# Project-Arda/bgls

Measured on AMD Instinct MI355X. Metric: aggregate-verify signer-pairs/sec, higher is better.
Workload: dtype u32; 1 GPU; altbn128 VerifyAggregateSignature, one 1048576-signer batch, keys+msgs resident in HBM; curve=altbn128, signers=1048576, signers_per_gpu=1048576, in_flight=8

## Files before the change

### bgls_amd/csrc/constants_gen.hpp

```cpp
#pragma once
#include <stdint.h>

namespace bgls {

struct BN254 {
  static constexpr int L = 8;
  static constexpr int CURVE_ID = 0;
  static constexpr bool TWIST_D = true;
  static constexpr int FP_BYTES = 32;
  static constexpr uint32_t N0INV = 0xe4866389u;
  static constexpr int XI_RE = 9;
  static constexpr uint32_t P[8] = {0xd87cfd47u, 0x3c208c16u, 0x6871ca8du, 0x97816a91u, 0x8181585du, 0xb85045b6u, 0xe131a029u, 0x30644e72u};
  static constexpr uint32_t P2W[16] = {0x275d69b1u, 0x3b5458a2u, 0x09eac101u, 0xa602072du, 0x6d96cadcu, 0x4a50189cu, 0x7a1242c8u, 0x04689e95u, 0x34c6b38du, 0x26edfa5cu, 0x16375606u, 0xb00b8551u, 0x0348d21cu, 0x599a6f7cu, 0x763cbf9cu, 0x0925c4b8u};
  static constexpr uint32_t P2W3[16] = {0x76183d13u, 0xb1fd09e6u, 0x1dc04303u, 0xf2061587u, 0x48c46095u, 0xdef049d5u, 0x6e36c858u, 0x0d39dbc0u, 0x9e541aa7u, 0x74c9ef14u, 0x42a60212u, 0x10228ff3u, 0x09da7656u, 0x0ccf4e74u, 0x62b63ed5u, 0x1b714e29u};
  static constexpr uint32_t P2W6[16] = {0xec307a26u, 0x63fa13ccu, 0x3b808607u, 0xe40c2b0eu, 0x9188c12bu, 0xbde093aau, 0xdc6d90b1u, 0x1a73b780u, 0x3ca8354eu, 0xe993de29u, 0x854c0424u, 0x20451fe6u, 0x13b4ecacu, 0x199e9ce8u, 0xc56c7daau, 0x36e29c52u};
  static constexpr uint32_t ONE[8] = {0xc58f0d9du, 0xd35d438du, 0xf5c70b3du, 0x0a78eb28u, 0x7879462cu, 0x666ea36fu, 0x9a07df2fu, 0x0e0a77c1u};
  static constexpr uint32_t R2[8] = {0x538afa89u, 0xf32cfc5bu, 0xd44501fbu, 0xb5e71911u, 0x0a417ff6u, 0x47ab1effu, 0xcab8351fu, 0x06d89f71u};
  static constexpr uint32_t HALF[8] = {0x4f060572u, 0x87bee7d2u, 0x2f1c6ae5u, 0xd0fd2addu, 0xfcfd4f44u, 0x8f5f7492u, 0x3d9cbfacu, 0x1f37631au};
  static constexpr uint32_t B[8] = {0x50ad28d7u, 0x7a17caa9u, 0xe15521b9u, 0x1f6ac17au, 0x696bd284u, 0x334bea4eu, 0xce179d8eu, 0x2a1f6744u};
  static constexpr uint32_t B2_RE[8] = {0x77b802a8u, 0x3bf938e3u, 0x3633535du, 0x020b1b27u, 0x49755260u, 0x26b7edf0u, 0x4384a86du, 0x2514c632u};
  static constexpr uint32_t B2_IM[8] = {0xd1dcff67u, 0x38e7ecccu, 0x93ce0d3eu, 0x65f0b37du, 0x22ac00aau, 0xd749d0ddu, 0x4a688d4du, 0x0141b9ceu};
  static constexpr uint32_t B2X3_RE[8] = {0xb62e0d6au, 0x3baa927cu, 0xd1b664fdu, 0xd71e7c52u, 0xd95d4664u, 0x03873e63u, 0x082ab8f4u, 0x0e75b5b1u};
  static constexpr uint32_t B2X3_IM[8] = {0x7596fe35u, 0xaab7c666u, 0xbb6a27bau, 0x31d21a78u, 0x680401ffu, 0x85dd7297u, 0xdf39a7e9u, 0x03c52d6au};
  static constexpr uint32_t GAMMA[288] = {0xc58f0d9du, 0xd35d438du, 0xf5c70b3du, 0x0a78eb28u, 0x7879462cu, 0x666ea36fu, 0x9a07df2fu, 0x0e0a77c1u, 0x00000000u, 0x00000000u, 0x00000000u, 0x00000000u, 0x00000000u, 0x00000000u, 0x00000000u, 0x00000000u, 0x33144907u, 0xaf9ba696u, 0x87afb78au, 0xca6b1d73u, 0xf08a2087u, 0x11bded5eu, 0x1a1f3a7cu, 0x02f34d75u, 0x4c492d72u, 0xa222ae23u, 0x565de15bu, 0xd00f02a4u, 0x53dfc926u, 0xdc2ff3a2u, 0xb3899551u, 0x10a75716u, 0x4563ab30u, 0xb5773b10u, 0xa9aa6454u, 0x347f91c8u, 0x242e0991u, 0x7a007127u, 0x118214ecu, 0x1956bcd8u, 0xa0aa4757u, 0x6e849f1eu, 0x89f89141u, 0xaa1c7b6du, 0xfae0ca3au, 0xb6e713cdu, 0x4e82ebc3u, 0x26694fbbu, 0x2936b629u, 0xe4bbdd0cu, 0xe133bacbu, 0xbb30f162u, 0xf9645366u, 0x31a9d1b6u, 0xa500f8ddu, 0x253570beu, 0x5ffe77c7u, 0xa1d77ce4u, 0x7826d1dbu, 0x07affd11u, 0xbb7edc6bu, 0x6d16bd27u, 0x85defeccu, 0x2c872002u, 0x843abe92u, 0x7361d77fu, 0x273411fbu, 0xa5bb2bd3u, 0x4b3e2399u, 0x9c941f31u, 0xbb9fd3ecu, 0x15df9cddu, 0x4bd8c949u, 0x5dddfd15u, 0xa4445b60u, 0x62cb29a5u, 0x0c7dd2b9u, 0x37bc870au, 0x3171f0fdu, 0x24830a9du, 0x41690fe7u, 0xc970692fu, 0x27694b0bu, 0xe2403421u, 0x83c459e8u, 0x32bee66bu, 0x0ab08841u, 0x12aabcedu, 0x40aebfa9u, 0x0d485d23u, 0xab2fcc57u, 0x05193418u, 0x8a4910f5u, 0xd3b0a40bu, 0x35d2925au, 0x2f21ebb5u, 0xc58f0d9du, 0xd35d438du, 0xf5c70b3du, 0x0a78eb28u, 0x7879462cu, 0x666ea36fu, 0x9a07df2fu, 0x0e0a77c1u, 0x00000000u, 0x00000000u, 0x00000000u, 0x00000000u, 0x00000000u, 0x00000000u, 0x00000000u, 0x00000000u, 0x00fa1bf2u, 0xca8d8005u, 0x68b39769u, 0xf0c5d614u, 0xad0d4418u, 0x0e201271u, 0xbad856e6u, 0x04290f65u, 0x00000000u, 0x00000000u, 0x00000000u, 0x00000000u, 0x00000000u, 0x00000000u, 0x00000000u, 0x00000000u, 0x13e80b9cu, 0x3350c88eu, 0xdb5e56b9u, 0x7dce557cu, 0xb615564au, 0x6001b4b8u, 0x020217e0u, 0x2682e617u, 0x00000000u, 0x00000000u, 0x00000000u, 0x00000000u, 0x00000000u, 0x00000000u, 0x00000000u, 0x00000000u, 0x12edefaau, 0x68c34889u, 0x72aabf4fu, 0x8d087f68u, 0x09081231u, 0x51e1a247u, 0x4729c0fau, 0x2259d6b1u, 0x00000000u, 0x00000000u, 0x00000000u, 0x00000000u, 0x00000000u, 0x00000000u, 0x00000000u, 0x00000000u, 0xd782e155u, 0x71930c11u, 0xffbe3323u, 0xa6bb947cu, 0xd4741444u, 0xaa303344u, 0x26594943u, 0x2c3b3f0du, 0x00000000u, 0x00000000u, 0x00000000u, 0x00000000u, 0x00000000u, 0x00000000u, 0x00000000u, 0x00000000u, 0xc494f1abu, 0x08cfc388u, 0x8d1373d4u, 0x19b31514u, 0xcb6c0213u, 0x584e90fdu, 0xdf2f8849u, 0x09e1685bu, 0x00000000u, 0x00000000u, 0x00000000u, 0x00000000u, 0x00000000u, 0x00000000u, 0x00000000u, 0x00000000u, 0xc58f0d9du, 0xd35d438du, 0xf5c70b3du, 0x0a78eb28u, 0x7879462cu, 0x666ea36fu, 0x9a07df2fu, 0x0e0a77c1u, 0x00000000u, 0x00000000u, 0x00000000u, 0x00000000u, 0x00000000u, 0x00000000u, 0x00000000u, 0x00000000u, 0x4e46d97du, 0x36531618u, 0xd4c96d9fu, 0x0af7129eu, 0xca1009b5u, 0x659da72fu, 0x83a20d23u, 0x08116d89u, 0xc39c1939u, 0xb1df4af7u, 0x8a73bf7fu, 0x3d9f0287u, 0x8caf0ae0u, 0x9b222092u, 0xeff054a6u, 0x26684515u, 0x16ad6badu, 0xc9af22f7u, 0x4aa662b2u, 0xb311782au, 0xe248c7f4u, 0x19eeaf64u, 0xe3439f82u, 0x20273e77u, 0xf7ce93acu, 0xacc02860u, 0x7ba76b4cu, 0x3933d581u, 0x446c8467u, 0x69e6188bu, 0x4417cc55u, 0x0a46036du, 0xaf46471eu, 0x5764af0au, 0x873e0fc1u, 0xdc50792eu, 0x881d04f6u, 0x86a673ffu, 0x3c30a74cu, 0x0b2eddb4u, 0x787e8580u, 0x9a490f32u, 0xf04af8b1u, 0x8fd16d7fu, 0xc6027bf2u, 0x4b39888eu, 0x5b52a15du, 0x03dd2e70u, 0x7b6762dfu, 0x448a93a5u, 0x28fdeadfu, 0xbfd62df5u, 0x0e9bd47au, 0xd858f5d0u, 0x3476ec58u, 0x06b03d4du, 0xbcc936d1u, 0x2b19daf4u, 0x56f4299fu, 0xa1a54e7au, 0x5adeaef1u, 0xb533eee0u, 0x84dda0b2u, 0x170c812bu, 0x75cf559fu, 0xe0bc4b22u, 0xc154e60fu, 0xc238b945u, 0x929a7d5eu, 0x803982a5u, 0xf7e4a37eu, 0x15ce052du, 0xbf3799a7u, 0x2d28efbdu, 0x1ad60773u, 0x9b097e3cu, 0xaf4a535bu, 0x982d4113u, 0xe3056063u, 0x24e18991u};
// ... 109 lines not shown
  static constexpr uint32_t RX_B2_RE[14] = {0x0d1ff2e0u, 0x06000000u, 0x000ac467u, 0x03379b48u, 0x01c84b80u, 0x00e88243u, 0x00dd9a7eu, 0x0683dcf8u, 0x06c26d0bu, 0x04a5eec2u, 0x0457663cu, 0x004b29f1u, 0x0967f3e8u, 0x00015de9u};
  static constexpr uint32_t RX_B2_IM[14] = {0x0d1ff2e0u, 0x06000000u, 0x000ac467u, 0x03379b48u, 0x01c84b80u, 0x00e88243u, 0x00dd9a7eu, 0x0683dcf8u, 0x06c26d0bu, 0x04a5eec2u, 0x0457663cu, 0x004b29f1u, 0x0967f3e8u, 0x00015de9u};
  static constexpr uint32_t RX_GAMMA[112] = {0x00000000u, 0x00000000u, 0x00000000u, 0x00000000u, 0x00000000u, 0x00000000u, 0x00000000u, 0x00000000u, 0x00000000u, 0x00000000u, 0x00000000u, 0x00000000u, 0x00000000u, 0x00000000u, 0x02421b59u, 0x0bee4867u, 0x01d31002u, 0x04760184u, 0x04cc5086u, 0x0c76dc00u, 0x0aae891bu, 0x0ac70ad2u, 0x0fe377c4u, 0x0e4686b8u, 0x05ed1568u, 0x08f5a180u, 0x002b5c1fu, 0x0000d1a4u, 0x033e2f27u, 0x032a25aau, 0x027ca1d2u, 0x0c1e049eu, 0x0c3f707au, 0x0055ca94u, 0x02010b7bu, 0x03b93794u, 0x0d5a86aau, 0x0a544de3u, 0x0556a044u, 0x09c66da5u, 0x038ec515u, 0x0000cea3u, 0x033e2f27u, 0x032a25aau, 0x027ca1d2u, 0x0c1e049eu, 0x0c3f707au, 0x0055ca94u, 0x02010b7bu, 0x03b93794u, 0x0d5a86aau, 0x0a544de3u, 0x0556a044u, 0x09c66da5u, 0x038ec515u, 0x0000cea3u, 0x0a75929au, 0x0681b798u, 0x022a3e9du, 0x0abc02bfu, 0x04e5bb45u, 0x055e6e7eu, 0x04814117u, 0x06d04f1bu, 0x0ae3387du, 0x054acb0cu, 0x00a4c74bu, 0x056138b5u, 0x0b64e066u, 0x000076f2u, 0x00000000u, 0x00000000u, 0x00000000u, 0x00000000u, 0x00000000u, 0x00000000u, 0x00000000u, 0x00000000u, 0x00000000u, 0x00000000u, 0x00000000u, 0x00000000u, 0x00000000u, 0x00000000u, 0x0cb7adf3u, 0x026fffffu, 0x03fd4ea0u, 0x0f320443u, 0x09b20bcbu, 0x01d54a7eu, 0x0f2fca33u, 0x019759edu, 0x0ac6b042u, 0x039151c5u, 0x0691dcb4u, 0x0e56da35u, 0x0b903c85u, 0x00014896u, 0x00000000u, 0x00000000u, 0x00000000u, 0x00000000u, 0x00000000u, 0x00000000u, 0x00000000u, 0x00000000u, 0x00000000u, 0x00000000u, 0x00000000u, 0x00000000u, 0x00000000u, 0x00000000u};
  static constexpr uint32_t RX_PK[126] = {0x00000000u, 0x00000000u, 0x00000000u, 0x00000000u, 0x00000000u, 0x00000000u, 0x00000000u, 0x00000000u, 0x00000000u, 0x00000000u, 0x00000000u, 0x00000000u, 0x00000000u, 0x00000000u, 0x0fffaaabu, 0x0fefffffu, 0x03ffffb9u, 0x0fffeb15u, 0x06241eabu, 0x0a0f6b0fu, 0x0f6730d2u, 0x0f38512bu, 0x04774b84u, 0x04bacd76u, 0x0ba7b643u, 0x0e69a4b1u, 0x01ea397fu, 0x0001a011u, 0x0fff5556u, 0x0fdfffffu, 0x07ffff73u, 0x0fffd62au, 0x0c483d57u, 0x041ed61eu, 0x0ece61a5u, 0x0e70a257u, 0x08ee9709u, 0x09759aecu, 0x074f6c86u, 0x0cd34963u, 0x03d472ffu, 0x00034022u, 0x0fff0001u, 0x0fcfffffu, 0x0bffff2du, 0x0fffc13fu, 0x026c5c03u, 0x0e2e412eu, 0x0e359277u, 0x0da8f383u, 0x0d65e28eu, 0x0e306862u, 0x02f722c9u, 0x0b3cee15u, 0x05beac7fu, 0x0004e033u, 0x0ffeaaacu, 0x0fbfffffu, 0x0ffffee7u, 0x0fffac54u, 0x08907aafu, 0x083dac3du, 0x0d9cc34au, 0x0ce144afu, 0x01dd2e13u, 0x02eb35d9u, 0x0e9ed90du, 0x09a692c6u, 0x07a8e5ffu, 0x00068044u, 0x0ffe5557u, 0x0fafffffu, 0x03fffea1u, 0x0fff976au, 0x0eb4995bu, 0x024d174cu, 0x0d03f41du, 0x0c1995dbu, 0x06547998u, 0x07a6034fu, 0x0a468f50u, 0x08103778u, 0x09931f7fu, 0x00082055u, 0x0ffe0002u, 0x0f9fffffu, 0x07fffe5bu, 0x0fff827fu, 0x04d8b807u, 0x0c5c825cu, 0x0c6b24efu, 0x0b51e707u, 0x0acbc51du, 0x0c60d0c5u, 0x05ee4593u, 0x0679dc2au, 0x0b7d58ffu, 0x0009c066u, 0x0ffdaaadu, 0x0f8fffffu, 0x0bfffe15u, 0x0fff6d94u, 0x0afcd6b3u, 0x066bed6bu, 0x0bd255c2u, 0x0a8a3833u, 0x0f4310a2u, 0x011b9e3bu, 0x0195fbd7u, 0x04e380dcu, 0x0d67927fu, 0x000b6077u, 0x0ffd5558u, 0x0f7fffffu, 0x0ffffdcfu, 0x0fff58a9u, 0x0120f55fu, 0x007b587bu, 0x0b398695u, 0x09c2895fu, 0x03ba5c27u, 0x05d66bb2u, 0x0d3db21au, 0x034d258du, 0x0f51cbffu, 0x000d0088u};
  static constexpr uint32_t RX_LAD[84] = {0x0fff5556u, 0x0fdfffffu, 0x07ffff73u, 0x0fffd62au, 0x0c483d57u, 0x041ed61eu, 0x0ece61a5u, 0x0e70a257u, 0x08ee9709u, 0x09759aecu, 0x074f6c86u, 0x0cd34963u, 0x03d472ffu, 0x00034022u, 0x0ffeaaacu, 0x0fbfffffu, 0x0ffffee7u, 0x0fffac54u, 0x08907aafu, 0x083dac3du, 0x0d9cc34au, 0x0ce144afu, 0x01dd2e13u, 0x02eb35d9u, 0x0e9ed90du, 0x09a692c6u, 0x07a8e5ffu, 0x00068044u, 0x0ffd5558u, 0x0f7fffffu, 0x0ffffdcfu, 0x0fff58a9u, 0x0120f55fu, 0x007b587bu, 0x0b398695u, 0x09c2895fu, 0x03ba5c27u, 0x05d66bb2u, 0x0d3db21au, 0x034d258du, 0x0f51cbffu, 0x000d0088u, 0x0ffaaab0u, 0x0effffffu, 0x0ffffb9fu, 0x0ffeb153u, 0x0241eabfu, 0x00f6b0f6u, 0x06730d2au, 0x038512bfu, 0x0774b84fu, 0x0bacd764u, 0x0a7b6434u, 0x069a4b1bu, 0x0ea397feu, 0x001a0111u, 0x0ff55560u, 0x0dffffffu, 0x0ffff73fu, 0x0ffd62a7u, 0x0483d57fu, 0x01ed61ecu, 0x0ce61a54u, 0x070a257eu, 0x0ee9709eu, 0x0759aec8u, 0x04f6c869u, 0x0d349637u, 0x0d472ffcu, 0x00340223u, 0x0feaaac0u, 0x0bffffffu, 0x0fffee7fu, 0x0ffac54fu, 0x0907aaffu, 0x03dac3d8u, 0x09cc34a8u, 0x0e144afdu, 0x0dd2e13cu, 0x0eb35d91u, 0x09ed90d2u, 0x0a692c6eu, 0x0a8e5ff9u, 0x00680447u};
};

struct BN254W : BN254 {
  static constexpr int RX_NL = 9;
  static constexpr int RX_W = 29;
  static constexpr uint32_t RX_MASK = 0x1fffffffu;
  static constexpr int RX_VBND = 4;
  static constexpr uint32_t RX_P[9] = {0x187cfd47u, 0x010460b6u, 0x1c72a34fu, 0x02d522d0u, 0x1585d978u, 0x02db40c0u, 0x00a6e141u, 0x0e5c2634u, 0x0030644eu};
  static constexpr uint32_t RX_NP = 0x4866389u;
  static constexpr uint32_t RX_ONE[9] = {0x157ccc21u, 0x141c2758u, 0x185230d3u, 0x014c0419u, 0x0aa36fb9u, 0x1d4240ceu, 0x11d54c07u, 0x052ac7a8u, 0x000dc836u};
  static constexpr uint32_t RX_R2[9] = {0x059bac10u, 0x0d1503a3u, 0x018016b8u, 0x10ab0ca8u, 0x02632639u, 0x02c0169fu, 0x169bfd53u, 0x11869d4cu, 0x002a11a6u};
  static constexpr uint32_t RX_TO[9] = {0x13349ca1u, 0x1a5d84a8u, 0x0a3e5cacu, 0x100249e0u, 0x12b951e8u, 0x0e92d304u, 0x14cb95b3u, 0x041b9d3du, 0x00058003u};
  static constexpr uint32_t RX_BACK[8] = {0x00000000u, 0x00000000u, 0x00000000u, 0x00000000u, 0x00000000u, 0x00000000u, 0x00000000u, 0x08000000u};
  static constexpr uint32_t RX_TOM[9] = {0x058f0d9du, 0x1aea1c6eu, 0x11c2cf74u, 0x11d651ebu, 0x1462c0a7u, 0x11b7bc3cu, 0x1cbd99bau, 0x183340fbu, 0x000e0a77u};
  static constexpr int RX_FAT_VB = 1;
  static constexpr int RX_FAT_KMAX = 6;
  static constexpr uint32_t RX_FAT[54] = {0x30f9fa8eu, 0x2208c16cu, 0x38e5469du, 0x25aa45a0u, 0x2b0bb2efu, 0x25b68180u, 0x214dc281u, 0x3cb84c67u, 0x0060c89bu, 0x4976f7d5u, 0x430d2222u, 0x5557e9ebu, 0x487f6870u, 0x40918c66u, 0x4891c240u, 0x41f4a3c1u, 0x4b14729au, 0x00912ce9u, 0x61f3f51cu, 0x641182d8u, 0x71ca8d39u, 0x6b548b40u, 0x761765ddu, 0x6b6d02ffu, 0x629b8501u, 0x797098cdu, 0x00c19136u, 0x9a70f263u, 0x8515e38du, 0x8e3d3087u, 0x8e29ae10u, 0x8b9d3f54u, 0x8e4843bfu, 0x83426641u, 0x87ccbf00u, 0x00f1f584u, 0xb2edefaau, 0xa61a4443u, 0xaaafd3d5u, 0xb0fed0e0u, 0xa12318cbu, 0xb123847fu, 0xa3e94781u, 0xb628e533u, 0x012259d1u, 0xcb6aecf1u, 0xc71ea4f9u, 0xc7227723u, 0xd3d3f3b0u, 0xd6a8f242u, 0xd3fec53eu, 0xc49028c1u, 0xc4850b66u, 0x0152be1fu};
  static constexpr uint64_t RX_BIAS_D3[18] = {0xbffffff6af4933bull, 0x17fffffeaa626d14ull, 0x23fffffdeceed0c9ull, 0x2ffffffd3de78d78ull, 0x3bfffffc65892178ull, 0x47fffffbaf384418ull, 0x53fffffaeef3e68aull, 0x5ffffffa2d17640aull, 0x54912ce7002863abull, 0x48912ce7c0000000ull, 0x3c912ce880000000ull, 0x30912ce940000000ull, 0x24912cea00000000ull, 0x18912ceac0000000ull, 0xc912ceb80000000ull, 0x912cec40000000ull, 0x1b71500000000ull, 0x0ull};
  static constexpr uint64_t RX_BIAS_S6[18] = {0x0ull, 0x0ull, 0x0ull, 0x0ull, 0x0ull, 0x0ull, 0x0ull, 0x0ull, 0x0ull, 0x0ull, 0x0ull, 0x0ull, 0x0ull, 0x0ull, 0x0ull, 0x0ull, 0x0ull, 0x0ull};
  static constexpr uint32_t RX_B2X3_RE[9] = {0x095cc5c1u, 0x016b1649u, 0x13202c16u, 0x05967b15u, 0x0b150904u, 0x0c884f0eu, 0x1423d855u, 0x02e3530fu, 0x001b2ff4u};
  static constexpr uint32_t RX_B2X3_IM[9] = {0x01e5cc12u, 0x15bda508u, 0x18588eb7u, 0x00f3e938u, 0x18f2b0b4u, 0x03bffebeu, 0x13752c37u, 0x0ec49a37u, 0x0017dd10u};
  static constexpr uint32_t RX_B2_RE[9] = {0x0b489658u, 0x00cfd255u, 0x0fdb9a77u, 0x02ce89f7u, 0x0033a0d4u, 0x1a768545u, 0x06ee3ddcu, 0x106a7dc1u, 0x0019316bu};
  static constexpr uint32_t RX_B2_IM[9] = {0x1b9fece0u, 0x07ecccd1u, 0x1069f1c7u, 0x0cdf64f3u, 0x0154cbe1u, 0x0dd22ac0u, 0x06eba4e8u, 0x1929a235u, 0x00283739u};
  static constexpr uint32_t RX_GAMMA[72] = {0x04a59190u, 0x06f504d9u, 0x0bf870bbu, 0x171ffd5cu, 0x1ac4d17du, 0x04be36d5u, 0x0bceec27u, 0x1a83a513u, 0x002492b3u, 0x11142ef1u, 0x0b31acc7u, 0x1d5818bcu, 0x180afc17u, 0x1a63177eu, 0x15765b3bu, 0x118f742eu, 0x063a509au, 0x00135e4eu, 0x1b1f0678u, 0x0373fb06u, 0x13170fbdu, 0x185d74b7u, 0x0241131fu, 0x16e18435u, 0x1ef3b6ceu, 0x01f06f02u, 0x001d46bdu, 0x19a647d5u, 0x19fdefabu, 0x1d925d1au, 0x0d1f6c5fu, 0x08ac6cc5u, 0x1fa5621au, 0x134f06feu, 0x09a72816u, 0x0015871du, 0x18ccb791u, 0x175b1c3au, 0x0b83d6e2u, 0x0e8ed071u, 0x1282bee2u, 0x04220e84u, 0x1fe4017fu, 0x15084d4au, 0x00169119u, 0x00000000u, 0x00000000u, 0x00000000u, 0x00000000u, 0x00000000u, 0x00000000u, 0x00000000u, 0x00000000u, 0x00000000u, 0x03003126u, 0x0ce8395eu, 0x0420727bu, 0x01891eb7u, 0x0ae269bfu, 0x0598fff2u, 0x0ed19539u, 0x09315e8bu, 0x00229c18u, 0x00000000u, 0x00000000u, 0x00000000u, 0x00000000u, 0x00000000u, 0x00000000u, 0x00000000u, 0x00000000u, 0x00000000u};
  static constexpr uint32_t RX_PK[81] = {0x00000000u, 0x00000000u, 0x00000000u, 0x00000000u, 0x00000000u, 0x00000000u, 0x00000000u, 0x00000000u, 0x00000000u, 0x187cfd47u, 0x010460b6u, 0x1c72a34fu, 0x02d522d0u, 0x1585d978u, 0x02db40c0u, 0x00a6e141u, 0x0e5c2634u, 0x0030644eu, 0x10f9fa8eu, 0x0208c16du, 0x18e5469eu, 0x05aa45a1u, 0x0b0bb2f0u, 0x05b68181u, 0x014dc282u, 0x1cb84c68u, 0x0060c89cu, 0x0976f7d5u, 0x030d2224u, 0x1557e9edu, 0x087f6872u, 0x00918c68u, 0x0891c242u, 0x01f4a3c3u, 0x0b14729cu, 0x00912cebu, 0x01f3f51cu, 0x041182dbu, 0x11ca8d3cu, 0x0b548b43u, 0x161765e0u, 0x0b6d0302u, 0x029b8504u, 0x197098d0u, 0x00c19139u, 0x1a70f263u, 0x0515e391u, 0x0e3d308bu, 0x0e29ae14u, 0x0b9d3f58u, 0x0e4843c3u, 0x03426645u, 0x07ccbf04u, 0x00f1f588u, 0x12edefaau, 0x061a4448u, 0x0aafd3dau, 0x10fed0e5u, 0x012318d0u, 0x11238484u, 0x03e94786u, 0x1628e538u, 0x012259d6u, 0x0b6aecf1u, 0x071ea4ffu, 0x07227729u, 0x13d3f3b6u, 0x16a8f248u, 0x13fec544u, 0x049028c7u, 0x04850b6cu, 0x0152be25u, 0x03e7ea38u, 0x082305b6u, 0x03951a78u, 0x16a91687u, 0x0c2ecbc0u, 0x16da0605u, 0x05370a08u, 0x12e131a0u, 0x01832273u};
  static constexpr uint32_t RX_LAD[54] = {0x10f9fa8eu, 0x0208c16du, 0x18e5469eu, 0x05aa45a1u, 0x0b0bb2f0u, 0x05b68181u, 0x014dc282u, 0x1cb84c68u, 0x0060c89cu, 0x01f3f51cu, 0x041182dbu, 0x11ca8d3cu, 0x0b548b43u, 0x161765e0u, 0x0b6d0302u, 0x029b8504u, 0x197098d0u, 0x00c19139u, 0x03e7ea38u, 0x082305b6u, 0x03951a78u, 0x16a91687u, 0x0c2ecbc0u, 0x16da0605u, 0x05370a08u, 0x12e131a0u, 0x01832273u, 0x07cfd470u, 0x10460b6cu, 0x072a34f0u, 0x0d522d0eu, 0x185d9781u, 0x0db40c0au, 0x0a6e1411u, 0x05c26340u, 0x030644e7u, 0x0f9fa8e0u, 0x008c16d8u, 0x0e5469e1u, 0x1aa45a1cu, 0x10bb2f02u, 0x1b681815u, 0x14dc2822u, 0x0b84c680u, 0x060c89ceu, 0x1f3f51c0u, 0x01182db0u, 0x1ca8d3c2u, 0x1548b438u, 0x01765e05u, 0x16d0302bu, 0x09b85045u, 0x17098d01u, 0x0c19139cu};
  static constexpr int64_t RX_XIG0[9] = {844385340ll, 595946497ll, 594944858ll, 816853286ll, 626800348ll, 805628652ll, 767515872ll, 770429518ll, -88799382ll};
  static constexpr int64_t RX_XIG1[9] = {274749216ll, 527690023ll, 296457758ll, 89892323ll, 256168189ll, 77064170ll, 186898397ll, 343619967ll, -101485007ll};
};

}
```

### bgls_amd/csrc/miller_x.hpp

```cpp
#pragma once
#include <type_traits>
#include "dev_common.hpp"
#include "coop.hpp"
#include "rx_pair.hpp"

namespace bgls {

template <class C>
struct MxForm { typedef C type; };
template <>
struct MxForm<BN254> { typedef BN254W type; };

template <class C, int NP = 60, bool XL_ = (std::is_same<C, BN254W>::value && NP == 60)>
struct MX {
  static_assert(NP == 60 || NP == 64, "pairings per block");
  static constexpr bool XL = XL_;
  static_assert(!XL || (NP == 60 && !rx_lazy<C> && C::TWIST_D && C::RX_NL <= 12), "XL: the 29-bit form's 60-pairing block, D-type twist");
  static constexpr int NL = C::RX_NL;
  static constexpr bool PACKED = (C::RX_NL % 4) != 0 && C::CURVE_ID == 1;
  static constexpr int HS = PACKED ? NL : ((NL + 3) & ~3);
  static constexpr int ES = 2 * HS;
  static constexpr int NLINES = NP == 64 ? 7 : 6;
  static constexpr int FOLD_UNROLL = (!rx_lazy<C> && NLINES % 3 == 0) ? 3 : 1;
  static constexpr int KS = PACKED ? 2 * ES : ES;
  static constexpr int WS = XL ? 112 : (PACKED ? 368 : 176);
  static constexpr int GROUP_DW = XL ? 1020 : (PACKED ? (NP == 64 ? 940 : 844) : (NP == 64 ? 828 : 764));
  static constexpr int THREADS = 192;
  static __device__ __forceinline__ int acc_off(int k, int wrap) { return k * KS + wrap * WS; }
  static __device__ __forceinline__ int line_off(int e) {
    if constexpr (PACKED) return e < 12 ? 28 + 56 * e + (e >= 6 ? 32 : 0) : (e == 12 ? 336 : 704 + 28 * (e - 13));
    else return 320 + ES * e;
  }
  static_assert(!PACKED || (ES == 28 && 704 + 28 * (3 * NLINES - 13) <= GROUP_DW), "BLS12-381 line slots");
  static_assert(PACKED || XL || 320 + ES * 3 * NLINES <= GROUP_DW, "alt-bn128 line slots");
  static __device__ __forceinline__ int line_off_x(int m, int t, bool xi, bool glo) {
    return t == 0 ? 256 + ES * m : (t == 1 ? (xi ? 544 + (glo ? 8 : 0) : 400) + ES * m : (xi ? 696 : 840) + ES * m);
  }
  static_assert(!XL || (ES == 24 && KS == 24 && WS + 3 * KS >= 6 * KS && WS + 6 * KS <= 256 && 840 + 6 * ES <= GROUP_DW), "XL line slots");
  static constexpr int PQ = 10 * GROUP_DW;
  static constexpr int P_LDS_LIMIT = 40960;
  static constexpr bool P_IN_LDS = (10 * GROUP_DW + NP * 2 * HS) * 4 <= P_LDS_LIMIT;
  static constexpr int BLOCK_BYTES = (10 * GROUP_DW + (P_IN_LDS ? NP * 2 * HS : 0)) * 4;
  static_assert(!XL || (BLOCK_BYTES <= 40960 && !P_IN_LDS), "XL: four blocks per CU; the hash points' coordinates are parked in the workspace");
  static constexpr int NPARK_Q = C::CURVE_ID == 0 ? 6 : 2;
  static constexpr int NPARK = NPARK_Q + (P_IN_LDS ? 0 : 2);
  static constexpr int PS = (NL + 3) & ~3;
  static constexpr size_t park_bytes(size_t nblocks) { return nblocks * 128 * NPARK * PS * 4; }
};

// ... 306 lines not shown
        const Sx<C, SX_T> b2 = sx_const<C>(odd ? C::RX_B2_IM : C::RX_B2_RE);
        const auto d = sx_sub<C>(pair_sqr<C>(yq, odd), sx_add<C>(pair_mul<C>(pair_sqr<C>(xq, odd), xq, odd), b2));
        const bool on_own = sx_is_zero_mod_p<C>(d);
        const bool on_curve = on_own && pair_swap1(on_own ? 1 : 0) != 0;
        if (valid && !(canon && (qinf || on_curve))) atomicOr(flags, FLAG_ENC);
      }
      Aff<F1<C>> P = g1s[valid ? idx : 0];
      valid = valid && !P.inf && !qinf;
      if (!valid) {
        xq = ux_to_sx<C>(to_ux<C>(fp_load<C>(C::G2 + (odd ? C::L : 0))));
        yq = ux_to_sx<C>(to_ux<C>(fp_load<C>(C::G2 + 2 * C::L + (odd ? C::L : 0))));
        P.x = fp_load<C>(C::G1X);
        P.y = fp_load<C>(C::G1Y);
      }
      MxPark<C>::st(mypark, 0, xq);
      MxPark<C>::st(mypark, 1, yq);
      if constexpr (C::CURVE_ID == 0) {
        const Sx<C, SX_T> cx = sx_select<C>(odd, sx_neg<C>(xq), xq), cy = sx_select<C>(odd, sx_neg<C>(yq), yq);
        constexpr int N2 = 2 * C::RX_NL;
        MxPark<C>::st(mypark, 2, pair_mul_const<C>(cx, C::RX_GAMMA + 0 * N2, C::RX_GAMMA + 0 * N2 + C::RX_NL, odd));
        MxPark<C>::st(mypark, 3, pair_mul_const<C>(cy, C::RX_GAMMA + 1 * N2, C::RX_GAMMA + 1 * N2 + C::RX_NL, odd));
        MxPark<C>::st(mypark, 4, pair_mul_const<C>(xq, C::RX_GAMMA + 2 * N2, C::RX_GAMMA + 2 * N2 + C::RX_NL, odd));
        MxPark<C>::st(mypark, 5, sx_norm<C>(sx_neg<C>(pair_mul_const<C>(yq, C::RX_GAMMA + 3 * N2, C::RX_GAMMA + 3 * N2 + C::RX_NL, odd))));
      }
      if constexpr (K::P_IN_LDS) {
        if (owner) mx_st_half<C, K::PACKED>(K::PQ + (2 * pi + (odd ? 1 : 0)) * K::HS, odd, odd ? to_ux<C>(P.x) : to_ux<C>(fp_neg<C>(P.y)));
        wave_sync();
      } else {
        MxPark<C>::st(mypark, P_NYP, ux_to_sx<C>(to_ux<C>(fp_neg<C>(P.y))));
        MxPark<C>::st(mypark, P_XP, ux_to_sx<C>(to_ux<C>(P.x)));
      }
      T.X = xq;
      T.Y = yq;
      T.Z = sx_select<C>(odd, ux_to_sx<C>(ux_zero<C>()), sx_const<C>(C::RX_ONE));
    }
    const int rl_base = tg * K::GROUP_DW + (odd ? K::HS : 0);
    Ux<C> e[K::XL ? 5 : 3];
    auto emit = [&](int which, const auto& v) __attribute__((always_inline)) {
      const int entry = which == 1 ? 1 : ((which == 0) == C::TWIST_D ? 0 : 2);
      if constexpr (rx_lazy<C>) e[entry] = sx_to_ux<C>(v);
      else if constexpr (std::is_same<std::decay_t<decltype(v)>, Sx<C, SX_T>>::value) e[entry] = sx_to_ux_p<C>(v);
      else e[entry] = sx_to_ux_k<1, C>(v);
      if constexpr (K::XL) {
        if (entry != 0) e[entry + 2] = pair_mulxi_half<C>(e[entry], odd);
      }
    };
    auto hand_over = [&]() __attribute__((always_inline)) {
      if (DBG == MX_DBG_CONSUMER || __builtin_amdgcn_ballot_w64(owner && !valid) != 0) {
        if (DBG == MX_DBG_CONSUMER || !valid) {
          e[0] = odd ? ux_zero<C>() : ux_load<C>(C::RX_ONE);
          e[1] = ux_zero<C>();
          e[2] = ux_zero<C>();
          if constexpr (K::XL) { e[3] = ux_zero<C>(); e[4] = ux_zero<C>(); }
        }
      }
      mx_stamp<DBG>(srec, 16 + 4 * sstep);
      __syncthreads();
      mx_stamp<DBG>(srec, 16 + 4 * sstep + 1);
      if (owner) {
        if constexpr (K::XL) {
#pragma unroll
          for (int t = 0; t < 3; ++t) mx_st_half<C, K::PACKED>(rl_base + K::line_off_x(m, t, false, tg < 6), odd, e[t]);
          mx_st_half<C, K::PACKED>(rl_base + K::line_off_x(m, 1, true, tg < 6), odd, e[3]);
          mx_st_half<C, K::PACKED>(rl_base + K::line_off_x(m, 2, true, tg < 6), odd, e[4]);
        } else {
          mx_st_half<C, K::PACKED>(rl_base + K::line_off(3 * m), odd, e[0]);
          mx_st_half<C, K::PACKED>(rl_base + K::line_off(3 * m + 1), odd, e[1]);
          mx_st_half<C, K::PACKED>(rl_base + K::line_off(3 * m + 2), odd, e[2]);
        }
      }
      mx_stamp<DBG>(srec, 16 + 4 * sstep + 2);
      __syncthreads();
      mx_stamp<DBG>(srec, 16 + 4 * sstep + 3);
      if constexpr (DBG == MX_DBG_STAMPS) ++sstep;
    };
    struct Env {
      const u32* pk;
      int xs, ys;
      bool neg_y;
      int pq;
      __device__ __forceinline__ Sx<C, SX_T> nyP() const {
        if constexpr (K::P_IN_LDS) return ux_to_sx<C>(mx_ld_half<C, K::PACKED>(pq, false));
        else return MxPark<C>::ld(MxPark<C>::launder(pk), K::NPARK_Q);
      }
      __device__ __forceinline__ Sx<C, SX_T> xP() const {
        if constexpr (K::P_IN_LDS) return ux_to_sx<C>(mx_ld_half<C, K::PACKED>(pq + K::HS, true));
        else return MxPark<C>::ld(MxPark<C>::launder(pk), K::NPARK_Q + 1);
      }
      __device__ __forceinline__ Sx<C, SX_T> xq() const { return MxPark<C>::ld(MxPark<C>::launder(pk), xs); }
      __device__ __forceinline__ Sx<C, SX_T> yq() const {
        const Sx<C, SX_T> y = MxPark<C>::ld(MxPark<C>::launder(pk), ys);
        return sx_select<C>(neg_y, sx_neg<C>(y), y);
      }
    };
#pragma unroll 1
    for (int i = 1; i < C::LOOP_LEN; ++i) {
      if constexpr (DBG != MX_DBG_CONSUMER) dbl_step_x<C>(T, Env{mypark, 0, 1, false, K::PQ + 2 * pi * K::HS}, odd, emit);
      hand_over();
      const int d = C::LOOP_NAF[i];
      if (d != 0) {
        if constexpr (DBG != MX_DBG_CONSUMER) add_step_x<C>(T, Env{mypark, 0, 1, d < 0, K::PQ + 2 * pi * K::HS}, odd, emit);
        hand_over();
      }
    }
    if constexpr (C::CURVE_ID == 0) {
#pragma unroll 1
      for (int s = 0; s < 2; ++s) {
        if constexpr (DBG != MX_DBG_CONSUMER) add_step_x<C>(T, Env{mypark, 2 + 2 * s, 3 + 2 * s, false, K::PQ + 2 * pi * K::HS}, odd, emit);
        hand_over();
      }
    }
    if constexpr (DBG == MX_DBG_NONE) {
      const bool z_own = sx_is_zero_mod_p<C>(T.Z);
      const bool z_zero = z_own && pair_swap1(z_own ? 1 : 0) != 0;
      if (valid && z_zero && !odd) atomicOr(flags, FLAG_DEGENERATE);
    }
  } else {
    if (rot_mode & 4) __builtin_amdgcn_s_setprio(3);
    const bool live = lane < 60;
    const int cl = live ? lane : lane - 12;
    const int g = cl % 10;
    const int j = cl / 10;
    const int gb = g * K::GROUP_DW;
    const bool glo = g < 6;
    Ux2<C> fj;
    {
      const Ux<C> one = ux_load<C>(C::RX_ONE);
#pragma unroll
      for (int k = 0; k < NL; ++k) { fj.c0.v[k] = j == 0 ? one.v[k] : 0u; fj.c1.v[k] = 0u; }
    }
    if constexpr (NP == 64) {
      if (live && g >= 4 && j < 3) {
        const Ux<C> one = ux_load<C>(C::RX_ONE), zero = ux_zero<C>();
        mx_st_half<C, K::PACKED>(gb + K::line_off(18 + j), false, j == 0 ? one : zero);
        mx_st_half<C, K::PACKED>(gb + K::line_off(18 + j) + K::HS, true, zero);
      }
    }
    mx_publish<C, NP>(gb, j, fj, live);
    unsigned sq_d = 0, sq_p = 0;
    if constexpr (!rx_lazy<C>) mx_sq_split(COOP_SQ_TAB[j], sq_d, sq_p);
    auto fold_all = [&](bool sq_next) __attribute__((always_inline)) {
// ... 58 lines not shown
```

### bgls_amd/csrc/rx.hpp

```cpp
#pragma once
#include "tower.hpp"

namespace bgls {

typedef int32_t i32;
typedef int64_t i64;
constexpr u32 RX_MASK = (1u << 28) - 1;
template <class C>
constexpr bool rx_lazy = 2 * C::RX_W + 8 <= 64;
template <class C>
constexpr bool rx_fits(long long budget) { return (long long)C::RX_NL * (budget + 256) + 64 < (1ll << (71 - 2 * C::RX_W)); }

#if !defined(__HIP_DEVICE_COMPILE__) && defined(BGLS_RX_CHECK)
extern int g_rx_overflow;
#define RX_HOST_CHECK 1
#else
#define RX_HOST_CHECK 0
#endif

BGLS_HD void rx_macu(u64& c, u32 a, u32 b) {
#if defined(__HIP_DEVICE_COMPILE__)
  asm volatile("v_mad_u64_u32 %0, vcc, %1, %2, %0" : "+v"(c) : "v"(a), "v"(b) : "vcc");
#elif RX_HOST_CHECK
  u64 r;
// ... 622 lines not shown
}

template <class C, int LA>
BGLS_HD Sx<C, SX_T> sx_quasi_center(const Sx<C, LA>& a) {
  constexpr int N = C::RX_NL;
  constexpr int W = C::RX_W;
  constexpr float QI = 1.0f / ((float)C::RX_P[N - 1] + 0.5f);
#if RX_HOST_CHECK
  {
    const i64 top = a.v[N - 1] < 0 ? -(i64)a.v[N - 1] : (i64)a.v[N - 1];
    if (top >= (1 << 24) || top > 64 * (i64)C::RX_P[N - 1] + 64) g_rx_overflow = 1;
  }
#endif
  const float qf = (float)a.v[N - 1] * QI;
  const i32 q = (i32)(qf + (qf < 0.0f ? -0.5f : 0.5f));
  Sx<C, SX_T> r;
  i64 c = 0;
#pragma unroll
  for (int i = 0; i < N - 1; ++i) {
    const i64 t = (i64)a.v[i] - (i64)q * (i64)(i32)C::RX_P[i] + c;
    r.v[i] = (i32)((u32)t & C::RX_MASK);
    c = t >> W;
  }
  r.v[N - 1] = (i32)((i64)a.v[N - 1] - (i64)q * (i64)(i32)C::RX_P[N - 1] + c);
#if RX_HOST_CHECK
  {
    const i64 top = r.v[N - 1] < 0 ? -(i64)r.v[N - 1] : (i64)r.v[N - 1];
    if (2 * top > (i64)C::RX_P[N - 1] + (i64)C::RX_P[N - 1] / 32 + 64) g_rx_overflow = 1;
  }
#endif
  return r;
}

template <class C, int LA>
BGLS_HD bool sx_is_zero_mod_p(const Sx<C, LA>& a) {
  constexpr int N = C::RX_NL;
  Sx<C, LA + 32> t;
#pragma unroll
  for (int i = 0; i < N; ++i) t.v[i] = a.v[i] + (i32)C::RX_PK[3 * N + i];
  const Sx<C, SX_T> n = sx_norm<C>(t);
  bool hit = false;
#pragma unroll
  for (int k = 0; k < 9; ++k) {
    u32 d = 0;
#pragma unroll
    for (int i = 0; i < N; ++i) d |= (u32)n.v[i] ^ C::RX_PK[k * N + i];
    hit = hit || d == 0;
  }
  return hit;
}
template <class C, int LA>
BGLS_HD bool sx_is_zero_mod_p_wide(const Sx<C, LA>& a) {
  constexpr int N = C::RX_NL;
  Sx<C, LA + 32> t;
#pragma unroll
  for (int i = 0; i < N; ++i) t.v[i] = a.v[i] + (i32)C::RX_PK[3 * N + i];
  Sx<C, SX_T> n = sx_norm<C>(t);
  if (n.v[N - 1] < 0 || n.v[N - 1] > (i32)C::RX_PK[8 * N + N - 1]) {
    const bool up = n.v[N - 1] < 0;
    Sx<C, LA + 48> u;
#pragma unroll
    for (int i = 0; i < N; ++i) u.v[i] = t.v[i] + (up ? (i32)C::RX_PK[8 * N + i] : -(i32)C::RX_PK[8 * N + i]);
    n = sx_norm<C>(u);
  }
  bool hit = false;
#pragma unroll
// ... 138 lines not shown
```

### bgls_amd/csrc/rx_pair.hpp

```cpp
#pragma once
#include "rx.hpp"

#if defined(__HIPCC__)
#define RX_DEV __device__ __forceinline__
#else
#define RX_DEV inline __attribute__((always_inline))
int rx_host_pair_swap(int v);
#endif

namespace bgls {

RX_DEV i32 pair_swap1(i32 v) {
#if defined(__HIPCC__)
  return __builtin_amdgcn_update_dpp(0, v, 0xB1 , 0xF, 0xF, true);
#else
  return rx_host_pair_swap(v);
#endif
}
RX_DEV i32 pair_even1(i32 v, bool odd) {
#if defined(__HIPCC__)
  (void)odd;
  return __builtin_amdgcn_update_dpp(0, v, 0xA0 , 0xF, 0xF, true);
#else
  const i32 o = rx_host_pair_swap(v);
// ... 103 lines not shown
  });
}
template <class C, int LG, int LE>
RX_DEV Sx<C, SX_T> pair_sqrsub3(const Sx<C, LG>& g, const Sx<C, LE>& e, bool odd) {
  static_assert(LG <= SX_F && LE <= SX_T, "g: a reduction's output or one carry step behind a sum; e: a reduction's output");
  constexpr int BUDGET = 513 + 6 * LE * LE;
  static_assert(rx_fits<C>(BUDGET), "two squares per reduction: 28-bit forms");
  Sx<C, 2 * LG> u;
  Sx<C, 2 * LE> w;
#pragma unroll
  for (int i = 0; i < C::RX_NL; ++i) {
    u.v[i] = g.v[i] + pair_odd1(g.v[i], odd);
    w.v[i] = e.v[i] + pair_odd1(e.v[i], odd);
  }
  const i32 even = odd ? 0 : -1;
  const i32* const cols[2] = {u.v, w.v};
  return sx_montr<C, 2, BUDGET>(cols, [&](int k, int i) {
    return k == 0 ? pair_even1(g.v[i], odd) - (pair_odd1(g.v[i], odd) & even) : -3 * (pair_even1(e.v[i], odd) - (pair_odd1(e.v[i], odd) & even));
  });
}
template <class C, int LA>
RX_DEV Sx<C, SX_T> pair_mul_3b(const Sx<C, LA>& z, bool odd) {
  if constexpr (C::CURVE_ID == 1) {
    static_assert(C::XI_RE == 1 && !C::TWIST_D, "3 b' = 12 (1 + i): BLS12-381's M-type twist");
    const auto t = sx_normf<C>(sx_add<C>(z, pair_swap_neg_even<C>(z, odd)));
    const auto t12 = sx_mulc<4, C>(sx_normf<C>(sx_mulc<3, C>(t)));
    return sx_quasi_center<C>(t12);
  } else {
    return pair_mul_const<C>(z, C::RX_B2X3_RE, C::RX_B2X3_IM, odd);
  }
}

template <class C>
struct PointX {
  Sx<C, SX_T> X, Y, Z;
};

template <class C, class T>
RX_DEV auto rx_nf(const T& a) {
  if constexpr (rx_lazy<C>) return a;
  else return sx_normf<C>(a);
}
template <class C, class Env, class Emit>
RX_DEV void dbl_step_x(PointX<C>& R, Env&& env, bool odd, Emit&& emit) {
  const Sx<C, SX_T> B = pair_sqr<C>(R.Y, odd);
  const Sx<C, SX_T> Cc = pair_sqr<C>(R.Z, odd);
  const auto H = rx_nf<C>(sx_sub<C>(pair_sqr<C>(sx_normf<C>(sx_add<C>(R.Y, R.Z)), odd), sx_add<C>(B, Cc)));
  const Sx<C, SX_T> E = pair_mul_3b<C>(Cc, odd);
  const auto J3 = rx_nf<C>(sx_mulc<3, C>(pair_sqr<C>(R.X, odd)));
  const auto A = rx_nf<C>(sx_half<C>(pair_mul<C>(R.X, R.Y, odd)));
  const Sx<C, SX_F> Fv = sx_normf<C>(sx_mulc<3, C>(E));
  R.X = pair_mul<C>(A, rx_nf<C>(sx_sub<C>(B, Fv)), odd);
  const Sx<C, SX_F> G = sx_normf<C>(sx_half<C>(sx_add<C>(B, Fv)));
  if constexpr (rx_lazy<C>) R.Y = pair_sqrsub3<C>(G, E, odd);
  else R.Y = sx_norm<C>(sx_sub<C>(pair_sqr<C>(G, odd), sx_mulc<3, C>(pair_sqr<C>(E, odd))));
  const auto I = sx_sub<C>(E, B);
  R.Z = pair_mul<C>(B, H, odd);
  emit(2, I);
  emit(0, pair_muls<C>(H, env.nyP()));
  emit(1, pair_muls<C>(J3, env.xP()));
}

template <class C, class Env, class Emit>
RX_DEV void add_step_x(PointX<C>& R, Env&& env, bool odd, Emit&& emit) {
  const Sx<C, SX_F> th = sx_normf<C>(sx_sub<C>(R.Y, pair_mul<C>(env.yq(), R.Z, odd)));
  const Sx<C, SX_F> la = sx_normf<C>(sx_sub<C>(R.X, pair_mul<C>(env.xq(), R.Z, odd)));
  const Sx<C, SX_T> D = pair_sqr<C>(la, odd);
  const Sx<C, SX_T> G = pair_mul<C>(R.X, D, odd);
  const Sx<C, SX_T> E = pair_mul<C>(la, D, odd);
  const Sx<C, SX_T> Fv = pair_mul<C>(R.Z, pair_sqr<C>(th, odd), odd);
  const Sx<C, SX_F> Hh = sx_normf<C>(sx_sub<C>(sx_add<C>(E, Fv), sx_mulc<2, C>(G)));
  R.X = pair_mul<C>(la, Hh, odd);
  R.Z = pair_mul<C>(R.Z, E, odd);
  if constexpr (rx_lazy<C>) {
    R.Y = pair_mulsub<C>(th, sx_sub<C>(G, Hh), E, R.Y, odd);
    emit(2, pair_mulsub<C>(th, env.xq(), la, env.yq(), odd));
  } else {
    R.Y = sx_norm<C>(sx_sub<C>(pair_mul<C>(th, sx_normf<C>(sx_sub<C>(G, Hh)), odd), pair_mul<C>(E, R.Y, odd)));
    emit(2, sx_sub<C>(pair_mul<C>(th, env.xq(), odd), pair_mul<C>(la, env.yq(), odd)));
  }
  emit(0, pair_muls<C>(sx_neg<C>(la), env.nyP()));
  emit(1, pair_muls<C>(sx_neg<C>(th), env.xP()));
}

}
```

Measured before the change: 19.03 million signer-pairs/s.

## Use xi-scaled projective Z in alt-bn128 Miller loop to cheapen 3b' multiply

For alt-bn128 on the 29-bit form, the Miller loop now keeps the projective Z coordinate scaled by xi^-1 (initialised to xi^-1). The general constant multiplication by 3b' in the doubling step becomes a cheap multiply by 9*xi using a small-constant reduction routine. To compensate, the add step multiplies Z by xi before use, and the yP line coefficient gets an extra xi multiply at emit time. The aim is to replace a full Fp2 constant multiply per doubling with small-integer operations, at the cost of extra xi multiplications in the add steps and emits.

```diff
diff --git a/bgls_amd/csrc/constants_gen.hpp b/bgls_amd/csrc/constants_gen.hpp
--- a/bgls_amd/csrc/constants_gen.hpp
+++ b/bgls_amd/csrc/constants_gen.hpp
@@ -165,6 +165,8 @@
   static constexpr uint32_t RX_LAD[54] = {0x10f9fa8eu, 0x0208c16du, 0x18e5469eu, 0x05aa45a1u, 0x0b0bb2f0u, 0x05b68181u, 0x014dc282u, 0x1cb84c68u, 0x0060c89cu, 0x01f3f51cu, 0x041182dbu, 0x11ca8d3cu, 0x0b548b43u, 0x161765e0u, 0x0b6d0302u, 0x029b8504u, 0x197098d0u, 0x00c19139u, 0x03e7ea38u, 0x082305b6u, 0x03951a78u, 0x16a91687u, 0x0c2ecbc0u, 0x16da0605u, 0x05370a08u, 0x12e131a0u, 0x01832273u, 0x07cfd470u, 0x10460b6cu, 0x072a34f0u, 0x0d522d0eu, 0x185d9781u, 0x0db40c0au, 0x0a6e1411u, 0x05c26340u, 0x030644e7u, 0x0f9fa8e0u, 0x008c16d8u, 0x0e5469e1u, 0x1aa45a1cu, 0x10bb2f02u, 0x1b681815u, 0x14dc2822u, 0x0b84c680u, 0x060c89ceu, 0x1f3f51c0u, 0x01182db0u, 0x1ca8d3c2u, 0x1548b438u, 0x01765e05u, 0x16d0302bu, 0x09b85045u, 0x17098d01u, 0x0c19139cu};
   static constexpr int64_t RX_XIG0[9] = {844385340ll, 595946497ll, 594944858ll, 816853286ll, 626800348ll, 805628652ll, 767515872ll, 770429518ll, -88799382ll};
   static constexpr int64_t RX_XIG1[9] = {274749216ll, 527690023ll, 296457758ll, 89892323ll, 256168189ll, 77064170ll, 186898397ll, 343619967ll, -101485007ll};
+  static constexpr uint32_t RX_XIINV_RE[9] = {0x16973135u, 0x0b46bbaeu, 0x041a1497u, 0x01e13998u, 0x1c9328c4u, 0x1f1b4201u, 0x0d31b509u, 0x1f978bfcu, 0x0018873du};
+  static constexpr uint32_t RX_XIINV_IM[9] = {0x13dff9a0u, 0x0d4eeef0u, 0x1acdfb42u, 0x044a76fbu, 0x0071994bu, 0x0f460e40u, 0x024e8c4du, 0x1db88b67u, 0x000d67bdu};
 };
 
 }
diff --git a/bgls_amd/csrc/miller_x.hpp b/bgls_amd/csrc/miller_x.hpp
--- a/bgls_amd/csrc/miller_x.hpp
+++ b/bgls_amd/csrc/miller_x.hpp
@@ -15,6 +15,7 @@
 struct MX {
   static_assert(NP == 60 || NP == 64, "pairings per block");
   static constexpr bool XL = XL_;
+  static constexpr bool ZXI = std::is_same<C, BN254W>::value;
   static_assert(!XL || (NP == 60 && !rx_lazy<C> && C::TWIST_D && C::RX_NL <= 12), "XL: the 29-bit form's 60-pairing block, D-type twist");
   static constexpr int NL = C::RX_NL;
   static constexpr bool PACKED = (C::RX_NL % 4) != 0 && C::CURVE_ID == 1;
@@ -387,15 +388,20 @@
       }
       T.X = xq;
       T.Y = yq;
-      T.Z = sx_select<C>(odd, ux_to_sx<C>(ux_zero<C>()), sx_const<C>(C::RX_ONE));
+      if constexpr (K::ZXI) T.Z = sx_const<C>(odd ? C::RX_XIINV_IM : C::RX_XIINV_RE);
+      else T.Z = sx_select<C>(odd, ux_to_sx<C>(ux_zero<C>()), sx_const<C>(C::RX_ONE));
     }
     const int rl_base = tg * K::GROUP_DW + (odd ? K::HS : 0);
     Ux<C> e[K::XL ? 5 : 3];
     auto emit = [&](int which, const auto& v) __attribute__((always_inline)) {
-      const int entry = which == 1 ? 1 : ((which == 0) == C::TWIST_D ? 0 : 2);
+      const bool yp = which == RX_EMIT_YP || which == RX_EMIT_YP_XI;
+      const int entry = which == 1 ? 1 : (yp == C::TWIST_D ? 0 : 2);
       if constexpr (rx_lazy<C>) e[entry] = sx_to_ux<C>(v);
       else if constexpr (std::is_same<std::decay_t<decltype(v)>, Sx<C, SX_T>>::value) e[entry] = sx_to_ux_p<C>(v);
       else e[entry] = sx_to_ux_k<1, C>(v);
+      if constexpr (K::ZXI) {
+        if (which == RX_EMIT_YP_XI) e[entry] = pair_mulxi_half<C>(e[entry], odd);
+      }
       if constexpr (K::XL) {
         if (entry != 0) e[entry + 2] = pair_mulxi_half<C>(e[entry], odd);
       }
@@ -450,18 +456,18 @@
     };
 #pragma unroll 1
     for (int i = 1; i < C::LOOP_LEN; ++i) {
-      if constexpr (DBG != MX_DBG_CONSUMER) dbl_step_x<C>(T, Env{mypark, 0, 1, false, K::PQ + 2 * pi * K::HS}, odd, emit);
+      if constexpr (DBG != MX_DBG_CONSUMER) dbl_step_x<C, K::ZXI>(T, Env{mypark, 0, 1, false, K::PQ + 2 * pi * K::HS}, odd, emit);
       hand_over();
       const int d = C::LOOP_NAF[i];
       if (d != 0) {
-        if constexpr (DBG != MX_DBG_CONSUMER) add_step_x<C>(T, Env{mypark, 0, 1, d < 0, K::PQ + 2 * pi * K::HS}, odd, emit);
+        if constexpr (DBG != MX_DBG_CONSUMER) add_step_x<C, K::ZXI>(T, Env{mypark, 0, 1, d < 0, K::PQ + 2 * pi * K::HS}, odd, emit);
         hand_over();
       }
     }
     if constexpr (C::CURVE_ID == 0) {
 #pragma unroll 1
       for (int s = 0; s < 2; ++s) {
-        if constexpr (DBG != MX_DBG_CONSUMER) add_step_x<C>(T, Env{mypark, 2 + 2 * s, 3 + 2 * s, false, K::PQ + 2 * pi * K::HS}, odd, emit);
+        if constexpr (DBG != MX_DBG_CONSUMER) add_step_x<C, K::ZXI>(T, Env{mypark, 2 + 2 * s, 3 + 2 * s, false, K::PQ + 2 * pi * K::HS}, odd, emit);
         hand_over();
       }
     }
diff --git a/bgls_amd/csrc/rx.hpp b/bgls_amd/csrc/rx.hpp
--- a/bgls_amd/csrc/rx.hpp
+++ b/bgls_amd/csrc/rx.hpp
@@ -678,6 +678,44 @@
   return r;
 }
 
+template <class C>
+BGLS_HD Sx<C, SX_T> sx_mul9xi_half(const Sx<C, SX_T>& a, const Sx<C, SX_T>& b, bool odd) {
+  static_assert(C::CURVE_ID == 0 && C::TWIST_D && C::XI_RE == 9, "9 xi = 81 + 9 i: alt-bn128's D-type twist");
+  constexpr int N = C::RX_NL;
+  constexpr int W = C::RX_W;
+  constexpr i32 KA = 9 * C::XI_RE, KB = 9;
+  constexpr float QI = 1.0f / ((float)C::RX_P[N - 1] + 0.5f);
+  static_assert((long long)(KA + KB) * 2 * ((long long)C::RX_P[N - 1] + 1) < (1ll << 31), "the top limbs' multiple stays a 32-bit value");
+#if RX_HOST_CHECK
+  for (int i = 0; i < N - 1; ++i)
+    if (a.v[i] < 0 || a.v[i] > (i32)C::RX_MASK || b.v[i] < 0 || b.v[i] > (i32)C::RX_MASK) g_rx_overflow = 1;
+  {
+    const i32 lo = -((i32)C::RX_P[N - 1] + 1), hi = 2 * ((i32)C::RX_P[N - 1] + 1);
+    if (a.v[N - 1] < lo || a.v[N - 1] > hi || b.v[N - 1] < lo || b.v[N - 1] > hi) g_rx_overflow = 1;
+  }
+#endif
+  const i32 kb = odd ? KB : -KB;
+  const i32 s = KA * a.v[N - 1] + kb * b.v[N - 1];
+  const i32 q = (i32)__builtin_rintf((float)s * QI);
+  Sx<C, SX_T> r;
+  i64 c = 0;
+#pragma unroll
+  for (int i = 0; i < N - 1; ++i) {
+    i64 t = (i64)KA * (i64)a.v[i] - (i64)q * (i64)(i32)C::RX_P[i] + c;
+    rx_macs(t, b.v[i], kb);
+    r.v[i] = (i32)((u32)t & C::RX_MASK);
+    c = t >> W;
+  }
+  r.v[N - 1] = s - q * (i32)C::RX_P[N - 1] + (i32)c;
+#if RX_HOST_CHECK
+  {
+    const i64 top = r.v[N - 1] < 0 ? -(i64)r.v[N - 1] : (i64)r.v[N - 1];
+    if (2 * top > (i64)C::RX_P[N - 1] + (i64)C::RX_P[N - 1] / 32 + 64) g_rx_overflow = 1;
+  }
+#endif
+  return r;
+}
+
 template <class C, int LA>
 BGLS_HD bool sx_is_zero_mod_p(const Sx<C, LA>& a) {
   constexpr int N = C::RX_NL;
diff --git a/bgls_amd/csrc/rx_pair.hpp b/bgls_amd/csrc/rx_pair.hpp
--- a/bgls_amd/csrc/rx_pair.hpp
+++ b/bgls_amd/csrc/rx_pair.hpp
@@ -159,21 +159,37 @@
 }
 
 template <class C>
+RX_DEV Sx<C, SX_T> pair_mul_9xi(const Sx<C, SX_T>& c, bool odd) {
+  Sx<C, SX_T> b;
+#pragma unroll
+  for (int i = 0; i < C::RX_NL; ++i) b.v[i] = pair_swap1(c.v[i]);
+  return sx_mul9xi_half<C>(c, b, odd);
+}
+template <class C>
+RX_DEV Sx<C, SX_T> pair_mulxi_sx(const Sx<C, SX_T>& u, bool odd) {
+  return ux_to_sx<C>(pair_mulxi_half<C>(sx_to_ux_p<C>(u), odd));
+}
+
+template <class C>
 struct PointX {
   Sx<C, SX_T> X, Y, Z;
 };
+constexpr int RX_EMIT_YP = 0, RX_EMIT_YP_XI = 3;
 
 template <class C, class T>
 RX_DEV auto rx_nf(const T& a) {
   if constexpr (rx_lazy<C>) return a;
   else return sx_normf<C>(a);
 }
-template <class C, class Env, class Emit>
+template <class C, bool ZXI = false, class Env, class Emit>
 RX_DEV void dbl_step_x(PointX<C>& R, Env&& env, bool odd, Emit&& emit) {
+  static_assert(!ZXI || (C::TWIST_D && C::CURVE_ID == 0 && !rx_lazy<C>), "the scaled form: alt-bn128 on the 29-bit form");
   const Sx<C, SX_T> B = pair_sqr<C>(R.Y, odd);
   const Sx<C, SX_T> Cc = pair_sqr<C>(R.Z, odd);
   const auto H = rx_nf<C>(sx_sub<C>(pair_sqr<C>(sx_normf<C>(sx_add<C>(R.Y, R.Z)), odd), sx_add<C>(B, Cc)));
-  const Sx<C, SX_T> E = pair_mul_3b<C>(Cc, odd);
+  Sx<C, SX_T> E;
+  if constexpr (ZXI) E = pair_mul_9xi<C>(Cc, odd);
+  else E = pair_mul_3b<C>(Cc, odd);
   const auto J3 = rx_nf<C>(sx_mulc<3, C>(pair_sqr<C>(R.X, odd)));
   const auto A = rx_nf<C>(sx_half<C>(pair_mul<C>(R.X, R.Y, odd)));
   const Sx<C, SX_F> Fv = sx_normf<C>(sx_mulc<3, C>(E));
@@ -184,18 +200,22 @@
   const auto I = sx_sub<C>(E, B);
   R.Z = pair_mul<C>(B, H, odd);
   emit(2, I);
-  emit(0, pair_muls<C>(H, env.nyP()));
+  emit(ZXI ? RX_EMIT_YP_XI : RX_EMIT_YP, pair_muls<C>(H, env.nyP()));
   emit(1, pair_muls<C>(J3, env.xP()));
 }
 
-template <class C, class Env, class Emit>
+template <class C, bool ZXI = false, class Env, class Emit>
 RX_DEV void add_step_x(PointX<C>& R, Env&& env, bool odd, Emit&& emit) {
-  const Sx<C, SX_F> th = sx_normf<C>(sx_sub<C>(R.Y, pair_mul<C>(env.yq(), R.Z, odd)));
-  const Sx<C, SX_F> la = sx_normf<C>(sx_sub<C>(R.X, pair_mul<C>(env.xq(), R.Z, odd)));
+  static_assert(!ZXI || (C::TWIST_D && C::CURVE_ID == 0 && !rx_lazy<C>), "the scaled form: alt-bn128 on the 29-bit form");
+  Sx<C, SX_T> Z;
+  if constexpr (ZXI) Z = pair_mulxi_sx<C>(R.Z, odd);
+  else Z = R.Z;
+  const Sx<C, SX_F> th = sx_normf<C>(sx_sub<C>(R.Y, pair_mul<C>(env.yq(), Z, odd)));
+  const Sx<C, SX_F> la = sx_normf<C>(sx_sub<C>(R.X, pair_mul<C>(env.xq(), Z, odd)));
   const Sx<C, SX_T> D = pair_sqr<C>(la, odd);
   const Sx<C, SX_T> G = pair_mul<C>(R.X, D, odd);
   const Sx<C, SX_T> E = pair_mul<C>(la, D, odd);
-  const Sx<C, SX_T> Fv = pair_mul<C>(R.Z, pair_sqr<C>(th, odd), odd);
+  const Sx<C, SX_T> Fv = pair_mul<C>(Z, pair_sqr<C>(th, odd), odd);
   const Sx<C, SX_F> Hh = sx_normf<C>(sx_sub<C>(sx_add<C>(E, Fv), sx_mulc<2, C>(G)));
   R.X = pair_mul<C>(la, Hh, odd);
   R.Z = pair_mul<C>(R.Z, E, odd);
```

Measured after the change: 19.20 million signer-pairs/s (median of 6 runs). About the same (+0.9%).
